# libAudioFlux/audioFlux

Hardware: AMD Instinct MI355X
Metric: audio frames/sec (mel+MFCC, n_fft=2048 hop=512) (higher is better)
Workload: dtype f32

## Files before the change

### audioflux_amd/csrc/hip/afx_melfused2.hip

```cpp
#include <hip/hip_runtime.h>

#include <cmath>
#include <cstdlib>
#include <cstring>

#include "afx_melplan.h"
#include "afx_melparts.h"
#include "afx_ccblock.h"

#ifdef AFX_V2_NTIN
#define AFX_V2_LOAD(p) __builtin_nontemporal_load(p)
#else
#define AFX_V2_LOAD(p) (*(p))
#endif
#ifndef AFX_V2_CCEVERY
#define AFX_V2_CCEVERY 16
#endif

namespace {

constexpr int NFFT = 2048;
constexpr int MC = 1024;
constexpr int WAVES = 12;
constexpr int WAVES_CPLX = 12;
__host__ __device__ constexpr int waves_of(bool cplx) { return cplx ? WAVES_CPLX : WAVES; }
constexpr int P1 = 72;
constexpr int PROW_OFF = 5120;
constexpr int PROW_F = 1104;
constexpr int WAVE_LDS = PROW_OFF + PROW_F * 4;
static_assert(16 * P1 * 8 <= PROW_OFF + 1025 * 4, "exchange image must end before the zero pad");
constexpr int T_WIN = 0;
constexpr int T_TW1 = 8192;
constexpr int T_TW2 = 16384;
constexpr int TW2_PITCH = 144;
constexpr int T_TW3 = 16960;
constexpr int T_BAND = 21056;
__host__ __device__ constexpr int wpitch(int ta, int tb) { return ta + tb + 4; }
__host__ __device__ constexpr int tab_bytes(int ta, int tb) { return T_BAND + 64 * wpitch(ta, tb) * 4; }
constexpr int DCT_PITCH = 36;
__host__ __device__ constexpr int block_lds_bytes(int ta, int tb, bool cc) {
    return tab_bytes(ta, tb) + (cc ? 64 * DCT_PITCH * 4 : 0) + WAVES * WAVE_LDS;
}

struct KArgs2 {
    const float *x;
    long long clipStride;
    long long totalFrames;
    int timeLength, hop;
    int framesPerWave;
    int aligned;
    const float4 *tab;
    const int *meta;
    int specMap, postPow;
    float normValue;
    float *out;
    float *outIm;
    int num;
    const float *dct;
    int ccNum, ccCbrt;
    float *cc;
    float *energy, *rms, *zcr;
    const float *win;
    int binLo, binCount;
    long long outPitch;
    int vecOut;
};


#ifndef AFX_PRIO_MASK
#define AFX_PRIO_MASK 0x1E
#endif
#ifndef AFX_PRIO_LEVEL
#define AFX_PRIO_LEVEL 1
#endif
#define MEL_PHASE(p)                                                                                       \
    do {                                                                                                   \
        if (AFX_PRIO_MASK != 0) __builtin_amdgcn_s_setprio(((AFX_PRIO_MASK >> (p)) & 1) ? AFX_PRIO_LEVEL : 0); \
    } while (0)

__device__ __forceinline__ float wave_sum(float v) {
#pragma unroll
    for (int o = 32; o > 0; o >>= 1) v += __shfl_xor(v, o, 64);
    return v;
}

template <int TA, int TB, int SHIFT, bool SPLIT, int CC, bool TEMPORAL, bool CPLX = false, bool STFT = false>
__global__ __launch_bounds__(waves_of(CPLX) * 64, 3) void k_stft_mel_v2(KArgs2 a) {
    constexpr int NWV = waves_of(CPLX);
    static_assert(!(CPLX && (CC || TEMPORAL)), "complex results: the bank only");
    static_assert(!STFT || (TA == 0 && TB == 0 && !SPLIT && CC == 0 && !TEMPORAL && !CPLX), "STFT instantiations: real rows, no bank");
    extern __shared__ __attribute__((aligned(16))) unsigned char smem[];
    const int lane = threadIdx.x & 63;
    const int wave = threadIdx.x >> 6;
    constexpr int WP = wpitch(TA, TB);
    constexpr int TABB = tab_bytes(TA, TB);
    constexpr int DCTB = CC == 1 ? 64 * DCT_PITCH * 4 : 0;
    unsigned char *wreg = smem + TABB + DCTB + wave * WAVE_LDS;
    float *prow = reinterpret_cast<float *>(wreg + PROW_OFF);

    {
        float4 *s4 = reinterpret_cast<float4 *>(smem);
        for (int i = threadIdx.x + (STFT ? T_TW1 / 16 : 0); i < TABB / 16; i += NWV * 64) s4[i] = a.tab[i];
        if constexpr (STFT) {
            v2 *tw = reinterpret_cast<v2 *>(smem + T_WIN);
            const v2 *w2 = reinterpret_cast<const v2 *>(a.win);
            for (int at = threadIdx.x; at < 1024; at += NWV * 64) {
                const int n1 = 2 * (at >> 7) + (at & 1), l = (at & 127) >> 1;
                tw[at] = w2[64 * n1 + l];
            }
        }
        if constexpr (CC == 1) {
            float *tabD = reinterpret_cast<float *>(smem + TABB);
            for (int i = threadIdx.x; i < 64 * 32; i += NWV * 64) {
                const int l = i >> 5, e = i & 31;
                const int fi = l & 15, g = l >> 4;
                tabD[l * DCT_PITCH + e] =
                    fi < a.ccNum ? a.dct[(long long)fi * a.num + 16 * (e >> 2) + 4 * g + (e & 3)] : 0.f;
            }
        }
        for (int i = 1025 + lane; i < PROW_F; i += 64) prow[i] = 0.f;
    }
    __syncthreads();

    const int k1 = lane >> 2, m2 = lane & 3;
    const unsigned T0 = lds_addr(smem), W0 = lds_addr(wreg);
    const unsigned aWin = T0 + T_WIN + 16 * lane;
    const unsigned aTw2 = T0 + T_TW2 + TW2_PITCH * m2;
    const unsigned aE1w = W0 + 8 * (8 * (k1 >> 1) + 2 * m2 + (k1 & 1));
    const unsigned aE1r = W0 + 576 * k1 + 16 * m2;
    const unsigned aE2w = W0 + 32 * k1 + 16 * ((m2 >> 1) ^ ((k1 >> 3) & 1)) + 8 * (m2 & 1);
    const int b3l = (lane >> 3) & 1;
    const unsigned aAlo = W0 + 32 * lane + 16 * b3l, aAhi = W0 + 32 * lane + 16 * (1 - b3l);
    const int qm0 = lane == 0 ? 128 : 256 - lane, qm1 = 192 - lane;
    const unsigned aB0lo = W0 + 32 * qm0 + 16 * ((qm0 >> 3) & 1), aB0hi = W0 + 32 * qm0 + 16 * (1 - ((qm0 >> 3) & 1));
    const unsigned aB1lo = W0 + 32 * qm1 + 16 * ((qm1 >> 3) & 1), aB1hi = W0 + 32 * qm1 + 16 * (1 - ((qm1 >> 3) & 1));
    const unsigned aT3lo = T0 + T_TW3 + 32 * lane + 16 * b3l, aT3hi = T0 + T_TW3 + 32 * lane + 16 * (1 - b3l);
    const unsigned R = W0 + PROW_OFF;
    const unsigned aP01 = R + 4 * lane;
    const unsigned aP23 = R + 4 * (lane == 0 ? 128 : lane + 512);
    const unsigned aQs1 = R + 4 * (192 - lane);
    const unsigned aQ23 = R + 4 * (lane == 0 ? 640 : 256 - lane);
    const bool lane0 = (lane == 0);

    const int startA = STFT ? 0 : a.meta[lane], startB = STFT ? 0 : a.meta[64 + lane];
    const int rowA = STFT ? -1 : a.meta[128 + lane], rowB = STFT ? -1 : a.meta[192 + lane];
    const unsigned seg0 = SPLIT ? (unsigned)a.meta[256 + lane] : 0u, seg1 = SPLIT ? (unsigned)a.meta[320 + lane] : 0u;
    const unsigned apa = R + 4 * startA, apb = R + 4 * startB;
    const unsigned awr = T0 + T_BAND + 4 * WP * lane;

    const long long gw = (long long)blockIdx.x * NWV + wave;
    long long f = gw * a.framesPerWave;
    long long fEnd = f + a.framesPerWave;
    if (fEnd > a.totalFrames) fEnd = a.totalFrames;
    if (f >= fEnd) return;
    int clip = (int)(f / a.timeLength);
    int t = (int)(f - (long long)clip * a.timeLength);
    int ccN = 0;

    v2 raw[16];
    auto fetch = [&](const float *px, int first) {
        if (a.aligned) {
            const v2 *p2 = reinterpret_cast<const v2 *>(px);
#pragma unroll
            for (int n1 = 0; n1 < 16; ++n1)
                if (n1 >= first) raw[n1] = AFX_V2_LOAD(&p2[64 * n1 + lane]);
        } else {
#pragma unroll
            for (int n1 = 0; n1 < 16; ++n1)
                if (n1 >= first) {
                    const int n = 64 * n1 + lane;
                    raw[n1] = v2{px[2 * n], px[2 * n + 1]};
                }
        }
    };
    fetch(a.x + (long long)clip * a.clipStride + (long long)t * a.hop, 0);

    auto cc_block = [&](long long fb, int cnt) {
        if constexpr (CC == 2) {
            ccb_rows<SPLIT ? 2 : 4>(a.out, a.cc, a.dct, a.num, a.ccNum, a.ccCbrt, fb, cnt, lane);
        } else {
        VM_WAIT_ALL();
        int ln = lane;
        PIN(ln);
        const int fi = ln & 15, g = ln >> 4;
        const long long r = fb + (fi < cnt ? fi : cnt - 1);
        const v4f *src = reinterpret_cast<const v4f *>(a.out + r * 128) + g;
        const unsigned ad = T0 + TABB + 4 * DCT_PITCH * ln;
        v4f acc[4] = {{0.f, 0.f, 0.f, 0.f}, {0.f, 0.f, 0.f, 0.f}, {0.f, 0.f, 0.f, 0.f}, {0.f, 0.f, 0.f, 0.f}};
        constexpr float LOG10_2 = 0.30102999566398120f;
#pragma unroll
        for (int h = 0; h < 2; ++h) {
            v4f av[4], dv[4];
#pragma unroll
            for (int u = 0; u < 4; ++u) LOAD_SC1_B128(av[u], src + 4 * (4 * h + u));
#pragma unroll
            for (int u = 0; u < 4; ++u) RD128(dv[u], ad, 16 * (4 * h + u));
            VM_LGKM_WAIT_ALL();
#pragma unroll
            for (int u = 0; u < 4; ++u) PIN(av[u]);
#pragma unroll
            for (int u = 0; u < 4; ++u) PIN(dv[u]);
#pragma unroll
            for (int u = 0; u < 4; ++u) {
#pragma unroll
                for (int c = 0; c < 4; ++c) {
                    const float lg = __log2f(fmaxf(av[u][c], 1e-8f)) * LOG10_2;
                    acc[c] = __builtin_amdgcn_mfma_f32_16x16x4f32(lg, dv[u][c], acc[c], 0, 0, 0);
                }
            }
        }
        const v4f sum = (acc[0] + acc[1]) + (acc[2] + acc[3]);
        if (fi < a.ccNum) {
#pragma unroll
            for (int reg = 0; reg < 4; ++reg) {
                const int rr = 4 * g + reg;
                if (rr < cnt) a.cc[(fb + rr) * a.ccNum + fi] = sum[reg];
            }
        }
        }
        ccN -= cnt;
    };

    for (; f < fEnd; ++f) {
        v2 v[16];
        MEL_PHASE(0);
        {
            v4f wv[8];
#pragma unroll
            for (int j = 0; j < 8; ++j) RD128_S(2, wv[j], aWin, T_WIN + 1024 * j);
            LDS_WAIT_N(4);
#pragma unroll
            for (int j = 0; j < 4; ++j) {
                PIN(wv[j]);
                v[2 * j] = raw[2 * j] * lo2(wv[j]);
                v[2 * j + 1] = raw[2 * j + 1] * hi2(wv[j]);
            }
            LDS_WAIT_N(0);
#pragma unroll
            for (int j = 4; j < 8; ++j) {
                PIN(wv[j]);
                v[2 * j] = raw[2 * j] * lo2(wv[j]);
                v[2 * j + 1] = raw[2 * j + 1] * hi2(wv[j]);
            }
        }
        if (f + 1 < fEnd) {
            int tn = t + 1, cn = clip;
            if (tn == a.timeLength) {
                tn = 0;
                ++cn;
            }
            const float *pn = a.x + (long long)cn * a.clipStride + (long long)tn * a.hop;
            bool whole = true;
            if constexpr (SHIFT > 0) {
                if (tn != 0) {
                    shift_rows_inplace<SHIFT>(raw);
                    fetch(pn, 16 - SHIFT);
                    whole = false;
                }
            }
            if (whole) fetch(pn, 0);
        }
        if constexpr (TEMPORAL) {
            float e = 0.f, z = 0.f;
            float prevTop = 0.f;
#pragma unroll
            for (int n1 = 0; n1 < 16; ++n1) {
                e = fmaf(v[n1].x, v[n1].x, e);
                e = fmaf(v[n1].y, v[n1].y, e);
                float py = __shfl_up(v[n1].y, 1, 64);
                if (lane0) py = prevTop;
                const bool first = (n1 == 0) && lane0;
                if (!first && v[n1].x * py < 0.f) z += 1.f;
                if (v[n1].y * v[n1].x < 0.f) z += 1.f;
                prevTop = __shfl(v[n1].y, 63, 64);
            }
            e = wave_sum(e);
            z = wave_sum(z);
            if (lane0) {
                a.energy[f] = e;
                a.rms[f] = sqrtf(e / (float)NFFT);
                a.zcr[f] = (float)((double)z / (double)NFFT);
            }
        }

        MEL_PHASE(1);
        dft16(v);
        {
            v4f tq[8];
#pragma unroll
            for (int j = 0; j < 8; ++j) RD128_S(2, tq[j], aWin, T_TW1 + 1024 * j);
            LDS_WAIT_N(0);
#pragma unroll
            for (int j = 0; j < 8; ++j) PIN(tq[j]);
            v2 o[16];
            o[0] = v[0];
#pragma unroll
            for (int k = 1; k < 16; ++k) o[k] = cmul(v[rev4(k)], (k & 1) ? hi2(tq[k >> 1]) : lo2(tq[k >> 1]));
#pragma unroll
            for (int g = 0; g < 4; ++g) {
                const unsigned b = aE1w + 2304 * g;
                WR2_64_S(0, b, o[4 * g], o[4 * g + 1], 0, 72);
                WR2_64_S(0, b, o[4 * g + 2], o[4 * g + 3], 144, 216);
            }
        }
        wave_lds_sync();
        MEL_PHASE(2);
        {
            v4f rq[8];
#pragma unroll
            for (int jj = 0; jj < 8; ++jj) RD128_S(1, rq[jj], aE1r, 64 * jj);
            wave_lds_sync();
#pragma unroll
            for (int jj = 0; jj < 8; ++jj) {
                PIN(rq[jj]);
                v[2 * jj] = lo2(rq[jj]);
                v[2 * jj + 1] = hi2(rq[jj]);
            }
        }

        MEL_PHASE(3);
        if (!KO_ON(5)) dft16(v);
        {
            v4f tq[8];
#pragma unroll
            for (int j = 0; j < 8; ++j) RD128_S(2, tq[j], aTw2, 16 * j);
            LDS_WAIT_N(0);
#pragma unroll
            for (int j = 0; j < 8; ++j) PIN(tq[j]);
            v2 o[16];
            o[0] = v[0];
#pragma unroll
            for (int j1 = 1; j1 < 16; ++j1) o[j1] = KO_ON(5) ? v[rev4(j1)] : cmul(v[rev4(j1)], (j1 & 1) ? hi2(tq[j1 >> 1]) : lo2(tq[j1 >> 1]));
#pragma unroll
            for (int g = 0; g < 4; ++g) {
                const unsigned b = aE2w + 2048 * g;
                WR2_64_S(0, b, o[4 * g], o[4 * g + 1], 0, 64);
                WR2_64_S(0, b, o[4 * g + 2], o[4 * g + 3], 128, 192);
            }
        }
        wave_lds_sync();

        MEL_PHASE(4);
        float pk[2][4], pq[2][4], p512;
        float ik[CPLX ? 2 : 1][4], iq[CPLX ? 2 : 1][4], i512 = 0.f;
        {
            v4f zalo[2], zahi[2], zblo[2], zbhi[2], wlo[2], whi[2];
            RD128_S(1, zalo[0], aAlo, 0);
            RD128_S(1, zahi[0], aAhi, 0);
            RD128_S(1, zblo[0], aB0lo, 0);
            RD128_S(1, zbhi[0], aB0hi, 0);
            RD128_S(2, wlo[0], aT3lo, 0);
            RD128_S(2, whi[0], aT3hi, 0);
            RD128_S(1, zalo[1], aAlo, 2048);
            RD128_S(1, zahi[1], aAhi, 2048);
            RD128_S(1, zblo[1], aB1lo, 0);
            RD128_S(1, zbhi[1], aB1hi, 0);
            RD128_S(2, wlo[1], aT3lo, 2048);
            RD128_S(2, whi[1], aT3hi, 2048);
#pragma unroll
            for (int s = 0; s < 2; ++s) {
                if (s == 0) LDS_WAIT_N(6);
                else LDS_WAIT_N(0);
                PIN(zalo[s]); PIN(zahi[s]); PIN(zblo[s]); PIN(zbhi[s]); PIN(wlo[s]); PIN(whi[s]);
                v2 za0 = lo2(zalo[s]), za1 = hi2(zalo[s]), za2 = lo2(zahi[s]), za3 = hi2(zahi[s]);
                v2 zb0 = lo2(zblo[s]), zb1 = hi2(zblo[s]), zb2 = lo2(zbhi[s]), zb3 = hi2(zbhi[s]);
                dft4(za0, za1, za2, za3);
                dft4(zb0, zb1, zb2, zb3);
                v2 A0 = za0, A1 = za1, A2 = za2, A3 = za3;
                v2 B0 = zb3, B1 = zb2, B2 = zb1, B3 = zb0;
                if (s == 0) {
                    if constexpr (CPLX) cplx_map(v2{za2.x, -za2.y}, a.specMap == 4, p512, i512);
                    else p512 = za2.x * za2.x + za2.y * za2.y;
                    A2 = lane0 ? zb0 : za2;
                    A3 = lane0 ? zb1 : za3;
                    B0 = lane0 ? za0 : zb3;
                    B1 = lane0 ? za3 : zb2;
                    B2 = lane0 ? zb3 : zb1;
                    B3 = lane0 ? zb2 : zb0;
                }
                if constexpr (CPLX) {
                    const bool sq = a.specMap == 4;
                    const v2 AA[4] = {A0, A1, A2, A3}, BB[4] = {B0, B1, B2, B3};
                    const v2 ww[4] = {lo2(wlo[s]), hi2(wlo[s]), lo2(whi[s]), hi2(whi[s])};
#pragma unroll
                    for (int j = 0; j < 4; ++j) {
                        v2 x, y;
                        split_pair_c(AA[j], BB[j], ww[j], x, y);
                        cplx_map(x, sq, pk[s][j], ik[CPLX ? s : 0][j]);
                        cplx_map(v2{y.x, -y.y}, sq, pq[s][j], iq[CPLX ? s : 0][j]);
                    }
                } else {
                    split_pair(A0, B0, lo2(wlo[s]), pk[s][0], pq[s][0]);
                    split_pair(A1, B1, hi2(wlo[s]), pk[s][1], pq[s][1]);
                    split_pair(A2, B2, lo2(whi[s]), pk[s][2], pq[s][2]);
                    split_pair(A3, B3, hi2(whi[s]), pk[s][3], pq[s][3]);
                }
            }
        }
        if constexpr (CPLX) {
            WR2ST_32(aP01 - PROW_OFF, ik[0][0], ik[0][1], 0, 4);
            WR2ST_32(aP23 - PROW_OFF, ik[0][2], ik[0][3], 0, 4);
            WR2ST_32(aP01 - PROW_OFF, ik[1][0], ik[1][1], 1, 5);
            WR2ST_32(aP01 - PROW_OFF, ik[1][2], ik[1][3], 9, 13);
            WR2ST_32(aQs1 - PROW_OFF, iq[0][1], iq[0][0], 9, 13);
            WR2ST_32(aQ23 - PROW_OFF, iq[0][3], iq[0][2], 0, 4);
            WR2ST_32(aQs1 - PROW_OFF, iq[1][3], iq[1][2], 0, 4);
            WR2ST_32(aQs1 - PROW_OFF, iq[1][1], iq[1][0], 8, 12);
            float *prowI = reinterpret_cast<float *>(wreg);
            if (lane0) prowI[512] = i512;
            prowI[1025 + lane] = 0.f;
            if (lane < PROW_F - 1025 - 64) prowI[1025 + 64 + lane] = 0.f;
        }
        WR2ST_32_S(4, aP01, pk[0][0], pk[0][1], 0, 4);
        WR2ST_32_S(4, aP23, pk[0][2], pk[0][3], 0, 4);
        WR2ST_32_S(4, aP01, pk[1][0], pk[1][1], 1, 5);
        WR2ST_32_S(4, aP01, pk[1][2], pk[1][3], 9, 13);
        WR2ST_32_S(4, aQs1, pq[0][1], pq[0][0], 9, 13);
        WR2ST_32_S(4, aQ23, pq[0][3], pq[0][2], 0, 4);
        WR2ST_32_S(4, aQs1, pq[1][3], pq[1][2], 0, 4);
        WR2ST_32_S(4, aQs1, pq[1][1], pq[1][0], 8, 12);
        if (lane0) prow[512] = p512;
        wave_lds_sync();
#pragma unroll
        for (int pass = 0; pass < (CPLX ? 2 : 1); ++pass) {
        const unsigned bpa = (CPLX && pass) ? apa - PROW_OFF : apa, bpb = (CPLX && pass) ? apb - PROW_OFF : apb;
        if (!CPLX && a.specMap) {
            for (int k = lane; k < 1025; k += 64) {
                const float p = prow[k];
                prow[k] = a.specMap == 1 ? sqrtf(p) : powf(p, a.normValue);
            }
            wave_lds_sync();
        }

        if constexpr (STFT) {
            MEL_PHASE(6);
            float *orow = a.out + f * a.outPitch;
            if (a.vecOut) {
                const float4 *p4 = reinterpret_cast<const float4 *>(prow);
                float4 *o4 = reinterpret_cast<float4 *>(orow);
                float4 q[4];
#pragma unroll
                for (int i = 0; i < 4; ++i) q[i] = p4[lane + 64 * i];
#pragma unroll
                for (int i = 0; i < 4; ++i) o4[lane + 64 * i] = q[i];
                if (lane0) o4[256] = p4[256];
            } else {
                for (int k = lane; k < a.binCount; k += 64) orow[k] = prow[a.binLo + k];
            }
        } else {
        MEL_PHASE(5);
        float accA, accB;
        {
            v2 sA, sB;
            band_stage<TA, TB, 4, CPLX>(awr, bpa, bpb, sA, sB);
            accA = sA.x + sA.y;
            accB = sB.x + sB.y;
        }
        if (!CPLX && !SPLIT && a.postPow) {
            accA = powf(accA, a.normValue);
            accB = powf(accB, a.normValue);
        }
        MEL_PHASE(6);
        if constexpr (CC != 0 && !SPLIT) {
            if (ccN == AFX_V2_CCEVERY) cc_block(f - AFX_V2_CCEVERY, AFX_V2_CCEVERY);
        }
        float *orow = ((CPLX && pass) ? a.outIm : a.out) + f * a.num;
        if constexpr (SPLIT) {
            float *part = reinterpret_cast<float *>(wreg + (CPLX ? PROW_F * 4 : 0));
            static_assert(PROW_F * 4 + 129 * 4 <= PROW_OFF, "segment sums must fit between the two rows");
            part[lane] = accA;
            part[64 + lane] = accB;
            if (lane0) part[128] = 0.f;
            wave_lds_sync();
#pragma unroll
            for (int h = 0; h < 2; ++h) {
                const unsigned u = h ? seg1 : seg0;
                float sum = part[u & 255u] + part[(u >> 8) & 255u];
                sum += part[(u >> 16) & 255u];
                sum += part[u >> 24];
                if (!CPLX && a.postPow) sum = powf(sum, a.normValue);
                if (lane + 64 * h < a.num) orow[lane + 64 * h] = sum;
            }
        } else {
            if (rowA >= 0) orow[rowA] = accA;
            if (rowB >= 0) orow[rowB] = accB;
        }
        if constexpr (CC != 0) {
            ++ccN;
            if (f + 1 == fEnd || (SPLIT && ccN == 16)) cc_block(f + 1 - ccN, ccN);
        }
        }
        wave_lds_sync();

        }

        if (++t == a.timeLength) {
            t = 0;
            ++clip;
        }
    }
}

void fill_tables(float *tab, const float *hWindow) {
    const double PI = 3.14159265358979323846;
    float *win = tab + T_WIN / 4, *tw1 = tab + T_TW1 / 4, *tw2 = tab + T_TW2 / 4, *tw3 = tab + T_TW3 / 4;
    for (int n1 = 0; n1 < 16; ++n1)
        for (int l = 0; l < 64; ++l) {
            const int at = 2 * (128 * (n1 >> 1) + 2 * l + (n1 & 1));
            const int n = 64 * n1 + l;
            if (hWindow) {
                win[at] = hWindow[2 * n];
                win[at + 1] = hWindow[2 * n + 1];
            }
            const double ang = -2.0 * PI * (double)(n1 * l) / MC;
            tw1[at] = (float)cos(ang);
            tw1[at + 1] = (float)sin(ang);
        }
    for (int m = 0; m < 4; ++m)
        for (int j = 0; j < 16; ++j) {
            const double ang = -2.0 * PI * (double)(m * j) / 64.0;
            tw2[(TW2_PITCH / 4) * m + 2 * j] = (float)cos(ang);
            tw2[(TW2_PITCH / 4) * m + 2 * j + 1] = (float)sin(ang);
        }
    for (int s = 0; s < 2; ++s)
        for (int l = 0; l < 64; ++l)
            for (int m = 0; m < 4; ++m) {
                int bin = l + 64 * s + 256 * m;
                if (s == 0 && l == 0 && m >= 2) bin = m == 2 ? 128 : 384;
                const double ang = -2.0 * PI * (double)bin / NFFT;
                const int at = 2 * (4 * (64 * s + l) + 2 * ((m >> 1) ^ ((l >> 3) & 1)) + (m & 1));
                tw3[at] = (float)(0.5 * cos(ang));
                tw3[at + 1] = (float)(0.5 * sin(ang));
            }
}

constexpr AfxMelVariant kVariants[] = {{48, 16}, {72, 32}};

template <int TA, int TB, int SHIFT, bool SPLIT, int CC, bool TEMPORAL, bool CPLX = false>
int launch_variant(const AfxMelPlan *p, const AfxMelFusedArgs *a, void *stream) {
    const long long total = (long long)a->batch * a->timeLength;
    if (total <= 0) return AFX_OK;
    constexpr int NWV = waves_of(CPLX);
    long long fpw;
    const long long blocks = afx_mel_frames(total, NWV, &fpw);

    KArgs2 k;
    memset(&k, 0, sizeof(k));
    k.x = a->x;
    k.clipStride = a->clipStride;
    k.totalFrames = total;
    k.timeLength = a->timeLength;
    k.hop = a->hop;
    k.framesPerWave = (int)fpw;
    k.aligned = ((a->clipStride & 1) == 0) && ((a->hop & 1) == 0) && ((reinterpret_cast<uintptr_t>(a->x) & 7) == 0);
    k.tab = reinterpret_cast<const float4 *>(p->dTab);
    k.meta = p->dMeta;
    k.specMap = a->specMap;
    k.postPow = a->postPow;
    k.normValue = a->normValue;
    k.out = a->out;
    k.outIm = a->outIm;
    k.num = p->num;
    k.dct = a->dct;
    k.ccNum = a->ccNum;
    k.ccCbrt = a->ccRectify == 1;
    k.cc = a->cc;
    k.energy = a->energy;
    k.rms = a->rms;
    k.zcr = a->zcr;
    constexpr size_t lds = (size_t)block_lds_bytes(TA, TB, CC == 1);
    static_assert(lds <= 163840, "workgroup LDS budget");
    AFX_LAUNCH_DYN_LDS((k_stft_mel_v2<TA, TB, SHIFT, SPLIT, CC, TEMPORAL, CPLX>), dim3((unsigned)blocks), dim3(NWV * 64), lds, stream, k);
    AFX_LAUNCH_CHECK("k_stft_mel_v2");
    return AFX_OK;
}

template <int TA, int TB, bool SPLIT, int CC, bool TEMPORAL>
int launch_hop(const AfxMelPlan *p, const AfxMelFusedArgs *a, void *stream) {
#ifdef AFX_EXPERIMENTS
    if (const char *e = getenv("AFX_EXP_MEL"))
        if (strstr(e, "noshift")) return launch_variant<TA, TB, 0, SPLIT, CC, TEMPORAL>(p, a, stream);
#endif
    switch (a->hop) {
        case 256: return launch_variant<TA, TB, 2, SPLIT, CC, TEMPORAL>(p, a, stream);
        case 512: return launch_variant<TA, TB, 4, SPLIT, CC, TEMPORAL>(p, a, stream);
        case 1024: return launch_variant<TA, TB, 8, SPLIT, CC, TEMPORAL>(p, a, stream);
        default: return launch_variant<TA, TB, 0, SPLIT, CC, TEMPORAL>(p, a, stream);
    }
}

template <int TA, int TB>
int launch(const AfxMelPlan *p, const AfxMelFusedArgs *a, void *stream) {
    const bool cc = a->cc != nullptr, tmp = a->energy != nullptr;
    if (a->specMap >= 3) {
        if (cc || tmp) return AFX_ERR_UNSUPPORTED;
        if (!a->outIm) return AFX_ERR_ARG;
        if (a->hop == 512)
            return p->split ? launch_variant<TA, TB, 4, true, 0, false, true>(p, a, stream)
                            : launch_variant<TA, TB, 4, false, 0, false, true>(p, a, stream);
        return p->split ? launch_variant<TA, TB, 0, true, 0, false, true>(p, a, stream)
                        : launch_variant<TA, TB, 0, false, 0, false, true>(p, a, stream);
    }
    if (cc && tmp) return AFX_ERR_UNSUPPORTED;
    if (cc) {
        if (a->ccNum < 1 || a->ccNum > 16 || !a->dct || !a->out || p->num > 128 || (p->num & 3)) return AFX_ERR_UNSUPPORTED;
        if (a->ccRectify != 0 && a->ccRectify != 1) return AFX_ERR_UNSUPPORTED;
        if constexpr (block_lds_bytes(TA, TB, true) <= 163840)
            if (!p->split && p->num == 128 && a->ccRectify == 0) return launch_hop<TA, TB, false, 1, false>(p, a, stream);
        if (a->hop == 512)
            return p->split ? launch_variant<TA, TB, 4, true, 2, false>(p, a, stream) : launch_variant<TA, TB, 4, false, 2, false>(p, a, stream);
        return p->split ? launch_variant<TA, TB, 0, true, 2, false>(p, a, stream) : launch_variant<TA, TB, 0, false, 2, false>(p, a, stream);
    }
    if (tmp) {
        if (!a->rms || !a->zcr) return AFX_ERR_ARG;
        return p->split ? launch_hop<TA, TB, true, 0, true>(p, a, stream)
                        : launch_hop<TA, TB, false, 0, true>(p, a, stream);
    }
    return p->split ? launch_hop<TA, TB, true, 0, false>(p, a, stream)
                    : launch_hop<TA, TB, false, 0, false>(p, a, stream);
}

int run(const AfxMelPlan *p, const AfxMelFusedArgs *a, void *stream) {
    return p->variant == 0 ? launch<48, 16>(p, a, stream) : launch<72, 32>(p, a, stream);
}

void fill_stft_tables(float *tab) { fill_tables(tab, nullptr); }

template <int SHIFT>
int launch_stft2k(const AfxStftArgs *a, const float *tab, void *stream) {
    const long long total = (long long)a->batch * a->timeLength;
    long long fpw;
    const long long blocks = afx_mel_frames(total, WAVES, &fpw);
    KArgs2 k;
    memset(&k, 0, sizeof(k));
    k.x = a->x;
    k.clipStride = a->clipStride;
    k.totalFrames = total;
    k.timeLength = a->timeLength;
    k.hop = a->hop;
    k.framesPerWave = (int)fpw;
    k.aligned = ((a->clipStride & 1) == 0) && ((a->hop & 1) == 0) && ((reinterpret_cast<uintptr_t>(a->x) & 7) == 0);
    k.tab = reinterpret_cast<const float4 *>(tab);
    k.specMap = a->mode == AFX_SPEC_POWER ? 0 : a->mode == AFX_SPEC_MAG ? 1 : 2;
    k.normValue = a->normValue;
    k.out = a->outRe;
    k.win = a->window;
    k.binLo = a->binLo;
    k.binCount = a->binCount;
    k.outPitch = a->outPitch ? a->outPitch : (long long)a->binCount;
    k.vecOut = a->binLo == 0 && a->binCount == NFFT / 2 + 1 && k.outPitch >= 1028 && (k.outPitch & 3) == 0 &&
               (reinterpret_cast<uintptr_t>(a->outRe) & 15) == 0;
    constexpr size_t lds = (size_t)block_lds_bytes(0, 0, false);
    AFX_LAUNCH_DYN_LDS((k_stft_mel_v2<0, 0, SHIFT, false, 0, false, false, true>), dim3((unsigned)blocks), dim3(WAVES * 64), lds, stream, k);
    AFX_LAUNCH_CHECK("k_stft_mel_v2 (stft)");
    return AFX_OK;
}

}

const AfxMelSize *afx_mel_size2k() {
    static const AfxMelSize size = {11, 0, kVariants, 2, T_BAND, fill_tables, run};
    return &size;
}

extern "C" int afxk_stft2k(const AfxStftArgs *a, void *stream) {
    if (a->radix2Exp != 11 || a->bandStart || a->energy || a->padLeft != 0 || a->hop < 1 || a->binLo < 0 || a->binCount < 1 ||
        a->binLo + a->binCount > NFFT / 2 + 1 || (long long)(a->timeLength - 1) * a->hop + NFFT > a->dataLength ||
        (reinterpret_cast<uintptr_t>(a->window) & 7) != 0)
        return AFX_ERR_UNSUPPORTED;
    if (a->mode != AFX_SPEC_POWER && a->mode != AFX_SPEC_MAG && a->mode != AFX_SPEC_POWER_NORM) return AFX_ERR_UNSUPPORTED;
    if (!a->outRe) return AFX_ERR_ARG;
    const long long total = (long long)a->batch * a->timeLength;
    if (total <= 0) return AFX_OK;
    if (total > 0x7fffffffLL) return AFX_ERR_UNSUPPORTED;
    const float *tab = afx_device_table<fill_stft_tables>((size_t)tab_bytes(0, 0));
    if (!tab) return AFX_ERR_UNSUPPORTED;
    switch (a->hop) {
        case 256: return launch_stft2k<2>(a, tab, stream);
        case 512: return launch_stft2k<4>(a, tab, stream);
        case 1024: return launch_stft2k<8>(a, tab, stream);
        default: return launch_stft2k<0>(a, tab, stream);
    }
}
```

Before: 683.0 million.

## Replace static per-wave frame split with per-workgroup dynamic claiming via LDS atomic

After: 698.7 million, median of 6. 1.02x the previous value.

```diff
diff --git a/audioflux_amd/csrc/hip/afx_melfused2.hip b/audioflux_amd/csrc/hip/afx_melfused2.hip
--- a/audioflux_amd/csrc/hip/afx_melfused2.hip
+++ b/audioflux_amd/csrc/hip/afx_melfused2.hip
@@ -15,6 +15,10 @@
 #endif
 #ifndef AFX_V2_CCEVERY
 #define AFX_V2_CCEVERY 16
+#endif
+#ifdef AFX_V2_STAMPS
+#include <cstdio>
+#include <vector>
 #endif
 
 namespace {
@@ -28,6 +32,7 @@
 constexpr int PROW_OFF = 5120;
 constexpr int PROW_F = 1104;
 constexpr int WAVE_LDS = PROW_OFF + PROW_F * 4;
+constexpr int CLAIM_LDS = 16;
 static_assert(16 * P1 * 8 <= PROW_OFF + 1025 * 4, "exchange image must end before the zero pad");
 constexpr int T_WIN = 0;
 constexpr int T_TW1 = 8192;
@@ -39,7 +44,13 @@
 __host__ __device__ constexpr int tab_bytes(int ta, int tb) { return T_BAND + 64 * wpitch(ta, tb) * 4; }
 constexpr int DCT_PITCH = 36;
 __host__ __device__ constexpr int block_lds_bytes(int ta, int tb, bool cc) {
-    return tab_bytes(ta, tb) + (cc ? 64 * DCT_PITCH * 4 : 0) + WAVES * WAVE_LDS;
+    return tab_bytes(ta, tb) + (cc ? 64 * DCT_PITCH * 4 : 0) + WAVES * WAVE_LDS + CLAIM_LDS;
+}
+
+__host__ __device__ constexpr int claim_length(int left, int waves, int minRun) {
+    const int g = left / (2 * waves);
+    if (left >= 16 * waves) return g >= 16 ? g & ~15 : 16;
+    return (g & ~3) > minRun ? g & ~3 : minRun;
 }
 
 struct KArgs2 {
@@ -47,7 +58,7 @@
     long long clipStride;
     long long totalFrames;
     int timeLength, hop;
-    int framesPerWave;
+    long long framesPerWg;
     int aligned;
     const float4 *tab;
     const int *meta;
@@ -64,7 +75,13 @@
     int binLo, binCount;
     long long outPitch;
     int vecOut;
+#ifdef AFX_V2_STAMPS
+    unsigned long long *stamps;
+#endif
 };
+#ifdef AFX_V2_STAMPS
+constexpr int STAMP_WORDS = 64, STAMP_HEAD = 8;
+#endif
 
 
 #ifndef AFX_PRIO_MASK
@@ -119,6 +136,7 @@
             }
         }
         for (int i = 1025 + lane; i < PROW_F; i += 64) prow[i] = 0.f;
+        if (threadIdx.x == 0) *reinterpret_cast<int *>(smem + TABB + DCTB + NWV * WAVE_LDS) = 0;
     }
     __syncthreads();
 
@@ -148,14 +166,44 @@
     const unsigned apa = R + 4 * startA, apb = R + 4 * startB;
     const unsigned awr = T0 + T_BAND + 4 * WP * lane;
 
-    const long long gw = (long long)blockIdx.x * NWV + wave;
-    long long f = gw * a.framesPerWave;
-    long long fEnd = f + a.framesPerWave;
-    if (fEnd > a.totalFrames) fEnd = a.totalFrames;
-    if (f >= fEnd) return;
-    int clip = (int)(f / a.timeLength);
-    int t = (int)(f - (long long)clip * a.timeLength);
+    const long long wgBeg = (long long)blockIdx.x * a.framesPerWg;
+    const int wgN = (int)(a.totalFrames - wgBeg < a.framesPerWg ? a.totalFrames - wgBeg : a.framesPerWg);
+    const int minRun = wgN >= 4 * NWV ? 4 : wgN > NWV ? (wgN + NWV - 1) / NWV : 1;
+    int *claimed = reinterpret_cast<int *>(smem + TABB + DCTB + NWV * WAVE_LDS);
+    const int wgClip = (int)(wgBeg / a.timeLength);
+    const unsigned wgT = (unsigned)(wgBeg - (long long)wgClip * a.timeLength);
+    auto locate = [&](long long fr, int &c, int &tt) {
+        const unsigned at = wgT + (unsigned)(fr - wgBeg);
+        c = wgClip + (int)(at / (unsigned)a.timeLength);
+        tt = (int)(at % (unsigned)a.timeLength);
+    };
+    auto claim = [&](long long &rb, long long &re) -> bool {
+        int s = wgN, l = 0;
+        if (lane0) {
+            const int left = wgN - __atomic_load_n(claimed, __ATOMIC_RELAXED);
+            if (left > 0) {
+                l = claim_length(left, NWV, minRun);
+                s = __atomic_fetch_add(claimed, l, __ATOMIC_RELAXED);
+            }
+        }
+        s = __builtin_amdgcn_readfirstlane(s);
+        l = __builtin_amdgcn_readfirstlane(l);
+        if (s >= wgN) return false;
+        rb = wgBeg + s;
+        re = wgBeg + (s + l < wgN ? s + l : wgN);
+        return true;
+    };
     int ccN = 0;
+#ifdef AFX_V2_STAMPS
+    unsigned long long *stamp = a.stamps + ((long long)blockIdx.x * NWV + wave) * STAMP_WORDS;
+    int stampN = 0;
+    if (lane0) {
+        stamp[0] = __builtin_amdgcn_s_memtime();
+        stamp[2] = (unsigned long long)blockIdx.x | ((unsigned long long)wave << 32);
+        stamp[4] = (unsigned)__builtin_amdgcn_s_getreg(4 | (0 << 6) | (31 << 11));
+        stamp[5] = (unsigned)__builtin_amdgcn_s_getreg(20 | (0 << 6) | (31 << 11));
+    }
+#endif
 
     v2 raw[16];
     auto fetch = [&](const float *px, int first) {
@@ -173,7 +221,6 @@
                 }
         }
     };
-    fetch(a.x + (long long)clip * a.clipStride + (long long)t * a.hop, 0);
 
     auto cc_block = [&](long long fb, int cnt) {
         if constexpr (CC == 2) {
@@ -221,6 +268,15 @@
         ccN -= cnt;
     };
 
+    long long fClaim, fEndClaim;
+    while (claim(fClaim, fEndClaim)) {
+    int laneZero = 0;
+    PIN(laneZero);
+    long long f = fClaim + laneZero;
+    const long long fEnd = fEndClaim;
+    int clip, t;
+    locate(fClaim, clip, t);
+    fetch(a.x + (long long)clip * a.clipStride + (long long)t * a.hop, 0);
     for (; f < fEnd; ++f) {
         v2 v[16];
         MEL_PHASE(0);
@@ -494,11 +550,22 @@
 
         }
 
+#ifdef AFX_V2_STAMPS
+        ++stampN;
+        if (lane0 && (stampN & 15) == 0 && STAMP_HEAD + (stampN >> 4) <= STAMP_WORDS) stamp[STAMP_HEAD - 1 + (stampN >> 4)] = __builtin_amdgcn_s_memtime();
+#endif
         if (++t == a.timeLength) {
             t = 0;
             ++clip;
         }
     }
+    }
+#ifdef AFX_V2_STAMPS
+    if (lane0) {
+        stamp[1] = __builtin_amdgcn_s_memtime();
+        stamp[3] = (unsigned long long)stampN;
+    }
+#endif
 }
 
 void fill_tables(float *tab, const float *hWindow) {
@@ -536,13 +603,48 @@
 
 constexpr AfxMelVariant kVariants[] = {{48, 16}, {72, 32}};
 
+long long wg_ranges(long long total, int waves, long long *framesPerWg) {
+    const char *e = getenv("AFX_MEL_CUS");
+    const int asked = e ? atoi(e) : 0;
+    const int cus = asked > 0 ? asked : afx_cu_count();
+    long long fpw;
+    long long blocks = afx_frame_split(total, cus, waves, 1, &fpw);
+    *framesPerWg = fpw * waves;
+    if (*framesPerWg > (1ll << 30)) {
+        *framesPerWg = 1ll << 30;
+        blocks = (total + *framesPerWg - 1) / *framesPerWg;
+    }
+    return blocks;
+}
+
+#ifdef AFX_V2_STAMPS
+unsigned long long *stamps_begin(long long blocks, int waves) {
+    unsigned long long *d = nullptr;
+    const size_t n = (size_t)blocks * waves * STAMP_WORDS * 8;
+    if (hipMalloc(&d, n) != hipSuccess || hipMemset(d, 0, n) != hipSuccess) return nullptr;
+    return d;
+}
+void stamps_end(unsigned long long *d, long long blocks, int waves, void *stream) {
+    const size_t n = (size_t)blocks * waves * STAMP_WORDS;
+    std::vector<unsigned long long> h(n);
+    (void)hipStreamSynchronize((hipStream_t)stream);
+    if (hipMemcpy(h.data(), d, n * 8, hipMemcpyDeviceToHost) == hipSuccess)
+        if (const char *name = getenv("AFX_V2_STAMPS_FILE"))
+            if (FILE *fp = fopen(name, "wb")) {
+                fwrite(h.data(), 8, n, fp);
+                fclose(fp);
+            }
+    (void)hipFree(d);
+}
+#endif
+
 template <int TA, int TB, int SHIFT, bool SPLIT, int CC, bool TEMPORAL, bool CPLX = false>
 int launch_variant(const AfxMelPlan *p, const AfxMelFusedArgs *a, void *stream) {
     const long long total = (long long)a->batch * a->timeLength;
     if (total <= 0) return AFX_OK;
     constexpr int NWV = waves_of(CPLX);
-    long long fpw;
-    const long long blocks = afx_mel_frames(total, NWV, &fpw);
+    long long fpg;
+    const long long blocks = wg_ranges(total, NWV, &fpg);
 
     KArgs2 k;
     memset(&k, 0, sizeof(k));
@@ -551,7 +653,7 @@
     k.totalFrames = total;
     k.timeLength = a->timeLength;
     k.hop = a->hop;
-    k.framesPerWave = (int)fpw;
+    k.framesPerWg = fpg;
     k.aligned = ((a->clipStride & 1) == 0) && ((a->hop & 1) == 0) && ((reinterpret_cast<uintptr_t>(a->x) & 7) == 0);
     k.tab = reinterpret_cast<const float4 *>(p->dTab);
     k.meta = p->dMeta;
@@ -570,8 +672,14 @@
     k.zcr = a->zcr;
     constexpr size_t lds = (size_t)block_lds_bytes(TA, TB, CC == 1);
     static_assert(lds <= 163840, "workgroup LDS budget");
+#ifdef AFX_V2_STAMPS
+    if (!(k.stamps = stamps_begin(blocks, NWV))) return AFX_ERR_HIP;
+#endif
     AFX_LAUNCH_DYN_LDS((k_stft_mel_v2<TA, TB, SHIFT, SPLIT, CC, TEMPORAL, CPLX>), dim3((unsigned)blocks), dim3(NWV * 64), lds, stream, k);
     AFX_LAUNCH_CHECK("k_stft_mel_v2");
+#ifdef AFX_V2_STAMPS
+    stamps_end(k.stamps, blocks, NWV, stream);
+#endif
     return AFX_OK;
 }
 
@@ -629,8 +737,8 @@
 template <int SHIFT>
 int launch_stft2k(const AfxStftArgs *a, const float *tab, void *stream) {
     const long long total = (long long)a->batch * a->timeLength;
-    long long fpw;
-    const long long blocks = afx_mel_frames(total, WAVES, &fpw);
+    long long fpg;
+    const long long blocks = wg_ranges(total, WAVES, &fpg);
     KArgs2 k;
     memset(&k, 0, sizeof(k));
     k.x = a->x;
@@ -638,7 +746,7 @@
     k.totalFrames = total;
     k.timeLength = a->timeLength;
     k.hop = a->hop;
-    k.framesPerWave = (int)fpw;
+    k.framesPerWg = fpg;
     k.aligned = ((a->clipStride & 1) == 0) && ((a->hop & 1) == 0) && ((reinterpret_cast<uintptr_t>(a->x) & 7) == 0);
     k.tab = reinterpret_cast<const float4 *>(tab);
     k.specMap = a->mode == AFX_SPEC_POWER ? 0 : a->mode == AFX_SPEC_MAG ? 1 : 2;
@@ -651,8 +759,14 @@
     k.vecOut = a->binLo == 0 && a->binCount == NFFT / 2 + 1 && k.outPitch >= 1028 && (k.outPitch & 3) == 0 &&
                (reinterpret_cast<uintptr_t>(a->outRe) & 15) == 0;
     constexpr size_t lds = (size_t)block_lds_bytes(0, 0, false);
+#ifdef AFX_V2_STAMPS
+    if (!(k.stamps = stamps_begin(blocks, WAVES))) return AFX_ERR_HIP;
+#endif
     AFX_LAUNCH_DYN_LDS((k_stft_mel_v2<0, 0, SHIFT, false, 0, false, false, true>), dim3((unsigned)blocks), dim3(WAVES * 64), lds, stream, k);
     AFX_LAUNCH_CHECK("k_stft_mel_v2 (stft)");
+#ifdef AFX_V2_STAMPS
+    stamps_end(k.stamps, blocks, WAVES, stream);
+#endif
     return AFX_OK;
 }
 
```
